# tlk00/BitMagic

Measured on AMD Instinct MI355X. Metric: Gbits/s + % HBM roofline, 256-way fused AND+COUNT on 1B-bit vectors, higher is better.
Workload: dtype u64; 1 GPU; aggregator pipeline combine_and_sub counts-only: 256-way AND+COUNT, 256 x 1000000000-bit vectors in total, data set A (common 10% OR noise 10%: no early exit); vectors=256, bits_per_vector=1000000000, density_q16=6554, blocks_per_vector=15259, blocks_per_rank=15259, hbm_resident_bytes=32279432448

## Files before the change

bitmagic_amd/__init__.py:

```python
from __future__ import annotations

import ctypes as C
from typing import Iterable, Sequence

import numpy as np

from . import _ffi
from ._ffi import BmxError, check, lib
from .sharding import shard_range, allreduce_counts

NULL, FULL, BIT, GAP = 0, 1, 2, 3
AND, OR, XOR, SUB = 0, 1, 2, 3
COUNT_AND, COUNT_XOR, COUNT_OR, COUNT_SUB_AB, COUNT_SUB_BA, COUNT_A, COUNT_B = 6, 7, 8, 9, 10, 11, 12
BLOCK_WORDS, BLOCK_BITS = 2048, 65536
opt_none, opt_compress = 0, 3
ID_MAX = 0xFFFFFFFF
ID_MAX64 = 0xFFFFFFFFFFFFFFFF
BM_UNSORTED, BM_SORTED, BM_SORTED_UNIFORM, BM_UNKNOWN = 0, 1, 2, 3

__all__ = ["context", "bvector", "aggregator", "slice_scanner", "rs_index", "rank_compressor", "group", "gbvector", "gaggregator", "gpipeline", "bit_import_u32", "count_and", "count_or",
           "count_xor", "count_sub", "distance_operation", "distance_matrix", "distance_matrix_dev",
           "COUNT_AND", "COUNT_XOR", "COUNT_OR", "COUNT_SUB_AB", "COUNT_SUB_BA", "COUNT_A", "COUNT_B", "BmxError", "simd_version", "device_count", "agg_run_options",
           "agg_opt_only_counts", "agg_opt_bvect_and_counts", "agg_opt_disable_bvects_and_counts",
           "BM_UNSORTED", "BM_SORTED", "BM_SORTED_UNIFORM", "BM_UNKNOWN"]
# ... 19 lines not shown
        self._h = C.c_void_p()
        check(lib().bmx_ctx_create(device, C.c_void_p(stream) if stream else None, C.byref(self._h)))
        self.device = device

    def close(self):
        if self._h:
            lib().bmx_ctx_destroy(self._h)
            self._h = C.c_void_p()

    def __del__(self):
        try:
            self.close()
        except Exception:
            pass

    def synchronize(self):
        check(lib().bmx_ctx_synchronize(self._h))

    def set_tuning(self, key: str, value: int):
        check(lib().bmx_ctx_set_tuning(self._h, key.encode(), int(value)))

    def trim(self):
        check(lib().bmx_ctx_trim(self._h))

    def redzone_check(self) -> dict:
        en, hits = C.c_int32(), C.c_uint64()
        buf = C.create_string_buffer(16384)
        check(lib().bmx_debug_redzone_check(self._h, C.byref(en), C.byref(hits), buf, len(buf)))
        return {"enabled": bool(en.value), "hits": hits.value, "report": buf.value.decode(errors="replace")}

    def inject_failure(self, kind: int, after: int = 0) -> None:
        check(lib().bmx_debug_inject_failure(self._h, int(kind), int(after)))

    def collection_prepare(self, vecs, role: int = 1) -> None:
        vecs = list(vecs)
        check(lib().bmx_collection_prepare(self._h, _handles(vecs), len(vecs), int(role)))

    def pack_stats(self) -> dict:
        n, b, ms = C.c_uint32(), C.c_uint64(), C.c_float()
        check(lib().bmx_ctx_pack_stats(self._h, C.byref(n), C.byref(b), C.byref(ms)))
        rb = C.c_uint64()
        check(lib().bmx_ctx_pack_run_bytes(self._h, C.byref(rb)))
        return {"collections": n.value, "bytes": b.value, "run_bytes": rb.value, "last_build_ms": ms.value}

    def mem_used(self) -> int:
        b = C.c_uint64()
# ... 1295 lines not shown
```

bitmagic_amd/_ffi.py:

```python
from __future__ import annotations

import ctypes as C
import os

_HERE = os.path.dirname(os.path.abspath(__file__))
LIB_PATH = os.environ.get("BMX_LIB") or os.path.join(_HERE, "lib", "libbmx.so")

OK, ERR_BADALLOC, ERR_BADARG, ERR_RANGE, ERR_DEVICE = 0, 1, 2, 3, 4


class BmxError(RuntimeError):
    def __init__(self, status: int, msg: str, detail: str):
        super().__init__(f"{msg}" + (f" [{detail}]" if detail else ""))
        self.status = status


_lib = None


def lib() -> C.CDLL:
    global _lib
    if _lib is not None:
        return _lib
    if not os.path.exists(LIB_PATH):
# ... 55 lines not shown
        "bmx_find_first_and_sub": (i32, [vp, P(vp), C.c_size_t, P(vp), C.c_size_t, P(i32), P(u64)]),
        "bmx_find_first_and_sub_range": (i32, [vp, P(vp), C.c_size_t, P(vp), C.c_size_t, u64, u64, P(i32), P(u64)]),
        "bmx_agg_shift_right_and": (i32, [vp, P(vp), C.c_size_t, i32, i32, P(vp), P(i32)]),
        "bmx_agg_shift_right_and_count": (i32, [vp, P(vp), C.c_size_t, P(u64)]),
        "bmx_slice_compare": (i32, [vp, P(vp), C.c_size_t, i32, u64, u64, u64, vp, P(vp), P(u64)]),
        "bmx_slice_compare_signed": (i32, [vp, P(vp), C.c_size_t, i32, C.c_int64, C.c_int64, u64, vp, P(vp), P(u64)]),
        "bmx_slice_compare_stat": (i32, [vp, P(vp), C.c_size_t, i32, u64, u64, u64, vp, P(u64), P(u64)]),
        "bmx_slice_eq_counts": (i32, [vp, P(vp), C.c_size_t, vp, C.c_size_t, u64, vp, vp]),
        "bmx_collection_prepare": (i32, [vp, P(vp), C.c_size_t, i32]),
        "bmx_ctx_pack_stats": (i32, [vp, P(u32), P(u64), P(C.c_float)]),
        "bmx_ctx_pack_run_bytes": (i32, [vp, P(u64)]),
        "bmx_pipeline_create": (i32, [vp, P(vp), P(u32), P(vp), P(u32), C.c_size_t, P(vp)]),
        "bmx_pipeline_destroy": (i32, [vp, vp]),
        "bmx_pipeline_set_search_count_limit": (i32, [vp, vp, u64]),
        "bmx_pipeline_last_windows": (i32, [vp, P(u32), P(u32)]),
        "bmx_pipeline_last_window_groups": (i32, [vp, P(u32), u32, P(u32)]),
        "bmx_pipeline_run_counts": (i32, [vp, vp, u32, u32, P(u64)]),
        "bmx_pipeline_run_counts_dev": (i32, [vp, vp, u32, u32, vp]),
        "bmx_pipeline_run_results": (i32, [vp, vp, P(vp), P(u64), vp, P(vp)]),
        "bmx_pipeline_run_results_range": (i32, [vp, vp, u32, u32, P(vp), P(u64), vp, P(vp)]),
        "bmx_pipeline_run_results_hint": (i32, [vp, vp, u64, u64, P(vp), P(u64), vp, P(vp)]),
        "bmx_pipeline_operand_bytes": (i32, [vp, vp, u32, u32, P(u64)]),
        "bmx_pipeline_describe": (i32, [vp, vp, u32, u32, C.c_char_p, C.c_size_t, P(u32)]),
        "bmx_rs_build": (i32, [vp, vp, P(vp)]),
        "bmx_rs_free": (i32, [vp, vp]),
        "bmx_rs_info": (i32, [vp, P(u64), P(i32)]),
        "bmx_rs_select_format": (i32, [vp, P(i32), P(u64)]),
        "bmx_rs_count": (i32, [vp, P(u64)]),
        "bmx_rs_export": (i32, [vp, vp, vp, vp]),
        "bmx_rank_batch": (i32, [vp, vp, vp, vp, C.c_size_t, vp]),
        "bmx_select_batch": (i32, [vp, vp, vp, vp, C.c_size_t, vp, vp]),
        "bmx_rank_batch_dev": (i32, [vp, vp, vp, vp, C.c_size_t, vp]),
        "bmx_select_batch_dev": (i32, [vp, vp, vp, vp, C.c_size_t, vp, vp]),
        "bmx_rank_compress": (i32, [vp, vp, vp, vp, i32, P(vp)]),
        "bmx_rank_decompress": (i32, [vp, vp, vp, vp, i32, P(vp)]),
        "bmx_rank_compress_many": (i32, [vp, vp, vp, P(vp), C.c_size_t, i32, P(vp)]),
        "bmx_rank_decompress_many": (i32, [vp, vp, vp, P(vp), C.c_size_t, i32, P(vp)]),
        "bmx_group_create": (i32, [P(i32), i32, i32, P(vp)]),
        "bmx_group_destroy": (i32, [vp]),
        "bmx_group_size": (i32, [vp, P(i32)]),
        "bmx_group_ctx": (i32, [vp, i32, P(vp)]),
        "bmx_group_shard_range": (i32, [vp, u32, i32, P(u32), P(u32)]),
        "bmx_block_table_weights": (i32, [u32, vp, vp, vp, u64, vp]),
        "bmx_group_partition_by_weight": (i32, [vp, u32, vp, vp]),
        "bmx_group_set_partition": (i32, [vp, u32, vp]),
        "bmx_group_rccl_ranks": (i32, [vp, P(i32)]),
# ... 67 lines not shown
```

bitmagic_amd/csrc/bmx.hip:

```cpp
#include "bmx_internal.h"
#ifdef BMX_DIAG
#include "bmx_diag.h"
#endif
#include "bmx_kernels2.h"
#include "bmx_kernels3.h"
#include "bmx_kernels4.h"
#include "bmx_kernels5.h"
#include "bmx_kernels6.h"
#include "bmx_kernels7.h"
#include "bmx_kernels8.h"
#include "bmx_kernels9.h"
#include "bmx_kernels10.h"
#include "bmx_kernels11.h"
#include "bmx_kernels12.h"
#include "bmx_kernels13.h"
#include "bmx_kernels14.h"
#include "bmx_kernels15.h"

#include <algorithm>
#include <atomic>
#include <chrono>
#include <cstdio>
#include <cstdlib>
#include <cstring>
// ... 627 lines not shown

static int coll_members_upload(bmx_ctx* ctx, const std::vector<u32>& ma, const std::vector<u32>& ms, DevBuf& d_buf, const u32** d_midx, const CollGroup** d_groups)
{
    const size_t nm = ma.size() + ms.size(), goff = (nm * 4 + 15) & ~(size_t)15;
    std::vector<u8> h(goff + sizeof(CollGroup));
    if (!ma.empty()) memcpy(h.data(), ma.data(), ma.size() * 4);
    if (!ms.empty()) memcpy(h.data() + ma.size() * 4, ms.data(), ms.size() * 4);
    const CollGroup g{0u, (u32)ma.size(), (u32)ma.size(), (u32)ms.size()};
    memcpy(h.data() + goff, &g, sizeof(g));
    int rc;
    if ((rc = dmalloc(ctx, &d_buf.p, h.size())) || (rc = h2d_staged(ctx, d_buf.p, h.data(), h.size()))) { d_buf.reset(); return rc; }
    *d_midx = (const u32*)d_buf.p; *d_groups = (const CollGroup*)((const char*)d_buf.p + goff);
    return BMX_OK;
}

static bool use_split(const bmx_ctx* ctx, const bmx_pipeline* p, u64 nitems)
{
    if (ctx->pipe_split == 0 || !nitems) return false;
    if (ctx->pipe_split == 1) return nitems <= 65535u * 16u;
    return nitems <= 384u && (u64)p->n_ops >= 24ull * p->ngroups;
}
#define SPLIT_WAVES 8

typedef void (*pipe_bits_fn)(const u64*, const u32*, const u32*, u32, u32, u32, u32, int, u64*);

static u32 pipe_window_cap(u32 wg)
{
    u32 wpb = wg / 64u;
    u32 per_cu = wpb >= 7u ? 1u : 12u / wpb;
    return 256u * per_cu * wpb;
}
static void pipe_plan(const bmx_ctx* ctx, u64 nitems, u32 ngroups, u32& rows, u32& wg, u32& unroll, u32& window)
{
    rows = (u32)ctx->pipe_rows;
    if (!rows) rows = nitems >= 1400u ? 8u : nitems >= 700u ? 4u : nitems >= 350u ? 2u : 1u;
    unroll = ctx->pipe_unroll ? (u32)ctx->pipe_unroll : ((rows >= 4u || !ctx->pipe_nt) ? 4u : 8u);
    u64 n = nitems * (8u / rows);
    wg = (u32)ctx->pipe_wg;
    if (!wg) {
        wg = 256u;
        if (rows == 8u) {
            static const u32 cand[3] = {640u, 768u, 512u};
            double best = -1.0;
            for (u32 c : cand) {
                u64 cap = pipe_window_cap(c), nwin = (n + cap - 1) / cap, per = (n + nwin - 1) / nwin;
                double fill = (double)per / (double)cap;
                if (fill > best + 0.02) { best = fill; wg = c; }
// ... 19 lines not shown
        if (unroll == 4 && nt) switch (wg) { case 384: return B2(4, true, 384); case 512: return B2(4, true, 512);
                                             case 640: return B2(4, true, 640); case 768: return B2(4, true, 768); default: break; }
        if (unroll == 4 && !nt && wg == 512) return B2(4, false, 512);
    }
#ifdef BMX_TUNE
    if constexpr (ROWS == 8) {
        if (nt && unroll == 4) switch (wg) { case 192: return B2(4, true, 192); case 320: return B2(4, true, 320); case 448: return B2(4, true, 448);
                                             case 576: return B2(4, true, 576); default: break; }
        if (nt && unroll == 2) switch (wg) { case 256: return B2(2, true, 256); case 384: return B2(2, true, 384); case 640: return B2(2, true, 640);
                                             case 1024: return B2(2, true, 1024); default: break; }
        if (nt && unroll == 1 && wg == 256) return B2(1, true, 256);
    } else {
        if (nt && wg == 384) {
            if (unroll == 4) return B2(4, true, 384);
            if constexpr (ROWS <= 4) { if (unroll == 8) return B2(8, true, 384); }
            if constexpr (ROWS <= 2) { if (unroll == 16) return B2(16, true, 384); }
        }
        if (nt && wg == 512 && unroll == 4) return B2(4, true, 512);
    }
#endif
#undef B2
    return nullptr;
}
static pipe_bits_fn pipe_bits_kernel(u32 rows, u32 unroll, bool nt, u32 wg)
{
    switch (rows) {
    case 8: return pipe_bits_rows<8>(unroll, nt, wg);
    case 4: return pipe_bits_rows<4>(unroll, nt, wg);
    case 2: return pipe_bits_rows<2>(unroll, nt, wg);
    case 1: return pipe_bits_rows<1>(unroll, nt, wg);
    default: return nullptr;
    }
}

static int ctx_set_tuning(bmx_ctx* ctx, const char* key, int value)
{
    ARGCHK(ctx && key);
    std::string k(key);
    if (k == "pipe_unroll") { ARGCHK(value == 0 || value == 1 || value == 2 || value == 4 || value == 8 || value == 16); ctx->pipe_unroll = value; }
    else if (k == "pipe_rows") { ARGCHK(value == 0 || value == 8 || value == 4 || value == 2 || value == 1); ctx->pipe_rows = value; }
    else if (k == "pipe_nt") ctx->pipe_nt = value != 0;
    else if (k == "pipe_lds") { ARGCHK(value >= 0 && value <= 160 * 1024); ctx->pipe_lds = value; }
    else if (k == "pipe_slots") { ARGCHK(value == 8 || value == 16); ctx->pipe_slots = value; }
    else if (k == "pipe_staged") { ARGCHK(value >= -1 && value <= 1); ctx->pipe_staged = value; }
    else if (k == "pipe_split") { ARGCHK(value >= -1 && value <= 1); ctx->pipe_split = value; }
    else if (k == "pipe_window") { ARGCHK(value >= -1); ctx->pipe_window = value; }
    else if (k == "or_tile") { ARGCHK(value >= 0 && value <= 3); ctx->or_tile = value; }
    else if (k == "or_rows") { ARGCHK(value >= -1 && value <= 1); ctx->or_rows = value; }
    else if (k == "or_depth") { ARGCHK(value == 4 || value == 8); ctx->or_depth = value; }
    else if (k == "direct_cols") { ARGCHK(value >= 0); ctx->direct_cols = value; }
    else if (k == "pair_stream") { ARGCHK(value == -1 || value == 0 || value == 2 || value == 4 || value == 8); ctx->pair_stream = value; }
    else if (k == "pair_wgs") { ARGCHK(value >= 1 && value <= 8); ctx->pair_wgs = value; }
    else if (k == "range_halves") { ARGCHK(value == 0 || value == 1); ctx->range_halves = value; }
    else if (k == "gap_count") { ARGCHK(value >= -1 && value <= 1); ctx->gap_count = value; }
    else if (k == "agg_shape") { ARGCHK(value == 0 || value == 1); ctx->agg_shape = value; }
    else if (k == "and_rows") { ARGCHK(value >= -1 && value <= 1); ctx->and_rows = value; }
    else if (k == "and_rows_wg") { ARGCHK(value == 128 || value == 256 || value == 512); ctx->and_rows_wg = value; }
    else if (k == "and_rows_depth") { ARGCHK(value == 2 || value == 3 || value == 4 || value == 8); ctx->and_rows_depth = value; }
    else if (k == "and_rows_nt") ctx->and_rows_nt = value != 0;
    else if (k == "and_rows_ipw") { ARGCHK(value >= 0 && value <= 64); ctx->and_rows_ipw = value; }
    else if (k == "ff_window") { ARGCHK(value >= -1); ctx->ff_window = value; }
    else if (k == "or_window") { ARGCHK(value >= -9); ctx->or_window = value; }
    else if (k == "gap_pack") { ARGCHK(value >= -1 && value <= 1); ctx->gap_pack = value; }
    else if (k == "coll_members") { ARGCHK(value >= -1 && value <= 1); ctx->coll_members = value; ++ctx->coll_gen; }
    else if (k == "coll_shape") { ARGCHK(value >= 0 && value <= 5); ctx->coll_shape = value; }
    else if (k == "op2_nt") { ARGCHK(value >= 0 && value <= 3); ctx->op2_nt = value; }
    else if (k == "op2_loop") { ARGCHK(value >= -1 && value <= 8); ctx->op2_loop = value; }
    else if (k == "op2_wgs") { ARGCHK(value >= 1 && value <= 8); ctx->op2_wgs = value; }
    else if (k == "pair_nt") { ARGCHK(value >= 0 && value <= 1); ctx->pair_nt = value; }
// ... 60 lines not shown
    dfree(ctx, p->scratch);
    const int rc = p->v ? vec_release(p->v) : BMX_OK;
    delete p;
    return rc;
}
void ctx_release(bmx_ctx* ctx)
{
    (void)hipSetDevice(ctx->device);
    if (ctx->stream) (void)hipStreamSynchronize(ctx->stream);
    while (!ctx->colls.empty()) coll_free(ctx, ctx->colls.size() - 1);
    pool_trim(ctx);
    rz_verify(ctx, nullptr);
    if (ctx->rz_hits) fprintf(stderr, "[bmx redzone] context destroyed with %llu damaged allocation(s) found during its life\n", (unsigned long long)ctx->rz_hits);
    for (auto& kv : ctx->pool_live) { auto rz = ctx->rz_live.find(kv.first); (void)hipFree(rz != ctx->rz_live.end() ? rz->second.raw : kv.first); if (rz != ctx->rz_live.end()) ctx->rz_live.erase(rz); }
    ctx->pool_live.clear();
    ensure_release(ctx, &ctx->scratch, &ctx->scratch_bytes);
    ensure_release(ctx, &ctx->aux, &ctx->aux_bytes);
    if (ctx->d_small) (void)hipFree(ctx->d_small);
    if (ctx->d_slots) (void)hipFree(ctx->d_slots);
    if (ctx->d_done) (void)hipFree(ctx->d_done);
    if (ctx->d_slots2) (void)hipFree(ctx->d_slots2);
    if (ctx->d_done2) (void)hipFree(ctx->d_done2);
    if (ctx->d_cursor) (void)hipFree(ctx->d_cursor);
    if (ctx->h_pend) (void)hipHostFree(ctx->h_pend);
    if (ctx->d_zero) (void)hipFree(ctx->d_zero);
    if (ctx->h_small) (void)hipHostFree(ctx->h_small);
    if (ctx->h_stage) (void)hipHostFree(ctx->h_stage);
    if (ctx->ev_stage) (void)hipEventDestroy(ctx->ev_stage);
    if (ctx->ev0) (void)hipEventDestroy(ctx->ev0);
    if (ctx->ev1) (void)hipEventDestroy(ctx->ev1);
    if (ctx->own_stream && ctx->stream) (void)hipStreamDestroy(ctx->stream);
    delete ctx;
}

extern "C" {

const char* bmx_error_msg(int status)
{
    switch (status) {
    case BMX_OK: return "BMX-00: All correct";
    case BMX_ERR_BADALLOC: return "BMX-01: Allocation error (HBM or host)";
    case BMX_ERR_BADARG: return "BMX-02: Invalid or missing function argument";
    case BMX_ERR_RANGE: return "BMX-03: Incorrect range or index";
    case BMX_ERR_DEVICE: return "BMX-04: No usable gfx950 device or HIP runtime failure";
    default: return "BMX-XX: Unknown error";
    }
// ... 20 lines not shown
    Owned<bmx_ctx> ctx(new bmx_ctx());
    ctx->device = device;
    if (stream) ctx->stream = (hipStream_t)stream;
    else { HIPCHK(hipStreamCreateWithFlags(&ctx->stream, hipStreamNonBlocking)); ctx->own_stream = true; }
    HIPCHK(hipEventCreate(&ctx->ev0));
    HIPCHK(hipEventCreate(&ctx->ev1));
    HIPCHK(hipMalloc((void**)&ctx->d_small, 64 * sizeof(u64)));
    HIPCHK(hipHostMalloc((void**)&ctx->h_small, 64 * sizeof(u64)));
    HIPCHK(hipHostMalloc((void**)&ctx->h_stage, STAGE_BYTES));
    HIPCHK(hipEventCreateWithFlags(&ctx->ev_stage, hipEventDisableTiming));
    HIPCHK(hipMalloc((void**)&ctx->d_slots, COUNT_SLOTS * COUNT_SLOT_STRIDE * sizeof(u64)));
    HIPCHK(hipMemsetAsync(ctx->d_slots, 0, COUNT_SLOTS * COUNT_SLOT_STRIDE * sizeof(u64), ctx->stream));
    HIPCHK(hipMalloc((void**)&ctx->d_zero, 256));
    HIPCHK(hipMemsetAsync(ctx->d_zero, 0, 256, ctx->stream));
    HIPCHK(hipMalloc((void**)&ctx->d_done, FOLD_DONE_WORDS * 4));
    HIPCHK(hipMemsetAsync(ctx->d_done, 0, FOLD_DONE_WORDS * 4, ctx->stream));
    HIPCHK(hipMalloc((void**)&ctx->d_slots2, COUNT_SLOTS * COUNT_SLOT_STRIDE * sizeof(u64)));
    HIPCHK(hipMemsetAsync(ctx->d_slots2, 0, COUNT_SLOTS * COUNT_SLOT_STRIDE * sizeof(u64), ctx->stream));
    HIPCHK(hipMalloc((void**)&ctx->d_done2, FOLD_DONE_WORDS * 4));
    HIPCHK(hipMemsetAsync(ctx->d_done2, 0, FOLD_DONE_WORDS * 4, ctx->stream));
    HIPCHK(hipHostMalloc((void**)&ctx->h_pend, PEND_SLOTS * 8 * sizeof(u64)));
    HIPCHK(hipMalloc((void**)&ctx->d_cursor, 64));
    HIPCHK(hipMemsetAsync(ctx->d_cursor, 0, 64, ctx->stream));
    { int v = 0; if (hipDeviceGetAttribute(&v, hipDeviceAttributeMaxSharedMemoryPerBlock, device) == hipSuccess && v > 0) ctx->max_lds_bytes = (uint32_t)v; else (void)hipGetLastError(); }
    { size_t fr = 0, tot = 0; if (hipMemGetInfo(&fr, &tot) == hipSuccess && fr) ctx->pack_cap = (uint64_t)fr / 4; else (void)hipGetLastError(); }
    if (const char* e = getenv("BMX_DEBUG_REDZONE")) ctx->redzone = atoi(e) != 0;
    if (const char* e = getenv("BMX_PACK_MAX_MB")) { long long mb = atoll(e); if (mb >= 0) ctx->pack_cap = (uint64_t)mb << 20; }
    if (const char* e = getenv("BMX_POOL_MAX_MB")) { long long mb = atoll(e); if (mb >= 0) ctx->pool_cap = (uint64_t)mb << 20; }
    static const char* const env_keys[][2] = {
        {"BMX_PIPE_UNROLL", "pipe_unroll"}, {"BMX_PIPE_ROWS", "pipe_rows"}, {"BMX_PIPE_NT", "pipe_nt"},
        {"BMX_PIPE_WG", "pipe_wg"}, {"BMX_PIPE_WINDOW", "pipe_window"}, {"BMX_PIPE_SPLIT", "pipe_split"}, {"BMX_OR_TILE", "or_tile"}, {"BMX_OR_ROWS", "or_rows"}, {"BMX_OR_DEPTH", "or_depth"}, {"BMX_OR_WINDOW", "or_window"}, {"BMX_DIRECT_COLS", "direct_cols"}, {"BMX_FF_WINDOW", "ff_window"}, {"BMX_GAP_COUNT", "gap_count"}, {"BMX_AND_ROWS", "and_rows"}, {"BMX_AGG_SHAPE", "agg_shape"}, {"BMX_AND_ROWS_WG", "and_rows_wg"}, {"BMX_AND_ROWS_DEPTH", "and_rows_depth"}, {"BMX_AND_ROWS_NT", "and_rows_nt"}, {"BMX_AND_ROWS_IPW", "and_rows_ipw"}, {"BMX_RANGE_HALVES", "range_halves"}, {"BMX_PAIR_STREAM", "pair_stream"}, {"BMX_PAIR_WGS", "pair_wgs"}, {"BMX_RS_LANES", "rs_lanes"}, {"BMX_RS_SELECT_TOP", "rs_select_top"}, {"BMX_RS_SELECT_SEL", "rs_select_sel"}, {"BMX_RS_LINES", "rs_lines"}, {"BMX_RS_SELECT_LINES", "rs_select_lines"}, {"BMX_RS_SDIR_SHIFT", "rs_sdir_shift"}, {"BMX_COLL_SHAPE", "coll_shape"}, {"BMX_COLL_WINDOW", "coll_window"}, {"BMX_COLL_SPLIT", "coll_split"}, {"BMX_COLL_BUILD", "coll_build"}, {"BMX_EQ_BIG", "eq_big"}, {"BMX_PAIR_LOOP", "pair_loop"}, {"BMX_PAIR_NT", "pair_nt"}, {"BMX_EQ_BIG_SHAPE", "eq_big_shape"}, {"BMX_OP2_WGS", "op2_wgs"}, {"BMX_OP2_LOOP", "op2_loop"}, {"BMX_OP2_NT", "op2_nt"}, {"BMX_GAP_PACK", "gap_pack"}, {"BMX_COLL_MEMBERS", "coll_members"}, {"BMX_XCD_SWIZZLE", "xcd_swizzle"}, {"BMX_RANKC_PATH", "rankc_path"}};
    for (auto& kv : env_keys)
        if (const char* e = getenv(kv[0])) (void)ctx_set_tuning(ctx.get(), kv[1], atoi(e));
    g_last_error.clear();
    *out = ctx.release();
    return BMX_OK;
ABI_END }

int bmx_ctx_destroy(bmx_ctx* ctx) { ABI_TRY if (ctx) ctx_release(ctx); return BMX_OK; ABI_END }

int bmx_ctx_set_tuning(bmx_ctx* ctx, const char* key, int value) { ABI_TRY return ctx_set_tuning(ctx, key, value); ABI_END }

int bmx_probe_stream_rw(bmx_ctx* ctx, uint64_t bytes, int sets, int wgs_per_cu, int iters, float* ms_per_pass)
{ ABI_TRY
    ARGCHK(ctx && ms_per_pass && bytes >= 8192 && sets >= 1 && sets <= 8 && wgs_per_cu >= 1 && wgs_per_cu <= 8 && iters >= 1);
    int rc = set_dev(ctx); if (rc) return rc;
    const u64 nblk = bytes / 8192;
    if (nblk > 0x7FFFFFFFull) { g_last_error = "probe buffer too large"; return BMX_ERR_RANGE; }
    void* buf = nullptr;
    HIPCHK(hipMalloc(&buf, (size_t)nblk * 8192 * 3 * sets));
    hipError_t e = hipMemsetAsync(buf, 0x5A, (size_t)nblk * 8192 * 3 * sets, ctx->stream);
    const u32 waves = 4u, total = 256u * waves * (u32)wgs_per_cu;
    const u32 per_wave = (u32)((nblk + total - 1u) / total);
    const u32 grid = (u32)(((nblk + per_wave - 1u) / per_wave + waves - 1u) / waves);
// ... 1169 lines not shown
        }
    }
    if (use_split(ctx, p, nitems64)) {
        size_t lds = (size_t)SPLIT_WAVES * 8192;
        auto fn = k_pipe_split<2, SPLIT_WAVES>;
        HIPCHK(hipFuncSetAttribute(reinterpret_cast<const void*>(fn), hipFuncAttributeMaxDynamicSharedMemorySize, (int)lds));
        hipLaunchKernelGGL(fn, dim3((u32)nitems64), dim3(SPLIT_WAVES * 64), lds, ctx->stream,
                           (const u64*)p->d_dmat, row_off, and_n, sub_n, p->col_stride, ngroups, nb_from, nb_to, 0, (u64*)d_counts,
                           0, (uint4*)nullptr, (u64*)nullptr, (BlockStat*)nullptr);
        KCHK();
        return BMX_OK;
    }
    if (!p->has_gap) {
        u32 rows, wg, unroll, window;
        pipe_plan(ctx, nitems64, ngroups, rows, wg, unroll, window);
        u32 parts = 8u / rows;
        if (nitems64 * parts > 0xFFFFFFF0ull) { g_last_error = "too many work items in one run"; return BMX_ERR_RANGE; }
        pipe_bits_fn fn = pipe_bits_kernel(rows, unroll, ctx->pipe_nt != 0, wg);
        if (!fn) { g_last_error = "this (pipe_rows, pipe_unroll, pipe_nt, pipe_wg) shape is not compiled into the library"; return BMX_ERR_BADARG; }
        u32 wpb = wg / 64u;
        u32 ncols = nb_to - nb_from;
        u32 nwin = window ? (ncols + window - 1u) / window : 1u;
        u32 per = (ncols + nwin - 1u) / nwin;
        for (u32 c0 = 0; c0 < ncols; c0 += per) {
            u32 cols = std::min(per, ncols - c0);
            u32 nitems = cols * ngroups * parts, grid = (nitems + wpb - 1) / wpb;
            hipLaunchKernelGGL(fn, dim3(grid), dim3(wg), (size_t)ctx->pipe_lds, ctx->stream,
                               (const u64*)p->d_dmat, row_off, and_n, p->col_stride, ngroups, nb_from + c0, nitems, ctx->xcd_swz, (u64*)d_counts);
            KCHK();
        }
        return BMX_OK;
    }
    if (nitems64 > 0xFFFFFFF0ull) { g_last_error = "too many (column, group) items in one run"; return BMX_ERR_RANGE; }
    if (use_and_rows(ctx, p)) {
        const u32 ipw = ctx->and_rows_ipw > 0 ? (u32)ctx->and_rows_ipw : 1u;
        hipLaunchKernelGGL(and_rows_kernel<AR_COUNT>(ctx), dim3((u32)((nitems64 + ipw - 1u) / ipw)), dim3((u32)ctx->and_rows_wg), 0, ctx->stream,
                           (const u64*)p->d_dmat, row_off, and_n, sub_n, p->col_stride, ngroups, nb_from, (u32)nitems64, ctx->xcd_swz, (u64*)d_counts,
                           (uint4*)nullptr, (u64*)nullptr, (BlockStat*)nullptr, 0u, 0xFFFFFFFFu, and_rows_diag_bits(), ipw);
        KCHK();
        return BMX_OK;
    }
    if (use_gapcount(ctx, p)) {
        size_t lds = (size_t)(16384 * 2 + 2048) * 4;
        HIPCHK(hipFuncSetAttribute(reinterpret_cast<const void*>(k_pipe_counts_gapcount<false>), hipFuncAttributeMaxDynamicSharedMemorySize, (int)lds));
        hipLaunchKernelGGL(HIP_KERNEL_NAME(k_pipe_counts_gapcount<false>), dim3((u32)nitems64), dim3(1024), lds, ctx->stream,
                           p->d_dmat, row_off, and_n, sub_n, p->col_stride, ngroups, nb_from, (u32)nitems64, (u64*)d_counts,
                           (uint4*)nullptr, (u64*)nullptr, (BlockStat*)nullptr, 0u, 0xFFFFFFFFu);
        KCHK();
        return BMX_OK;
    }
    size_t lds = 4 * 2048 * 4;
// ... 35 lines not shown
        snprintf(buf, buf_len, "k_pipe_split<2,%d> x 1 launch, %llu workgroups", SPLIT_WAVES, (unsigned long long)nitems64);
    else if (use_and_rows(ctx, p))
        snprintf(buf, buf_len, "k_agg_and_rows<COUNT,%d,%d> x 1 launch, %llu workgroups", ctx->and_rows_wg, ctx->and_rows_depth, (unsigned long long)nitems64);
    else if (use_gapcount(ctx, p))
        snprintf(buf, buf_len, "k_pipe_counts_gapcount x 1 launch, %llu workgroups", (unsigned long long)nitems64);
    else if (p->has_gap)
        snprintf(buf, buf_len, "k_pipe_counts<%d> x 1 launch", ctx->pipe_unroll == 1 ? 1 : ctx->pipe_unroll == 2 ? 2 : 4);
    else {
        u32 rows, wg, unroll, window;
        pipe_plan(ctx, nitems64, p->ngroups, rows, wg, unroll, window);
        u32 ncols = nb_to - nb_from, nwin = (window && ncols) ? (ncols + window - 1u) / window : 1u;
        u32 per = nwin ? (ncols + nwin - 1u) / nwin : 0u;
        snprintf(buf, buf_len, "k_pipe_counts_bits2<%u,%s,%u,%u> x %u launch%s of <= %u columns", unroll, ctx->pipe_nt ? "true" : "false",
                 wg, rows, nwin, nwin == 1 ? "" : "es", per);
        if (n_launches) *n_launches = nwin;
    }
    return BMX_OK;
ABI_END }

int bmx_pipeline_set_search_count_limit(bmx_ctx* ctx, bmx_pipeline* p, uint64_t limit)
{ ABI_TRY
    ARGCHK(ctx && p && p->ctx == ctx);
    p->search_limit = (limit == 0 || limit == 0xFFFFFFFFull || limit == 0xFFFFFFFFFFFFull) ? ~0ull : limit;
    return BMX_OK;
ABI_END }

int bmx_pipeline_last_windows(const bmx_pipeline* p, uint32_t* launched, uint32_t* planned)
{ ABI_TRY
    ARGCHK(p);
    if (launched) *launched = p->last_windows;
    if (planned) *planned = p->last_windows_planned;
    return BMX_OK;
ABI_END }

}

static int limit_counts_run(bmx_ctx* ctx, bmx_pipeline* p, uint32_t nb_from, uint32_t nb_to, uint64_t* counts_out)
{
    int rc;
    uint32_t f = nb_from, t = nb_to;
    if ((rc = pipe_range(p, f, t))) return rc;
    const u32 ng = p->ngroups, ncols = t - f;
    p->h_win_groups.clear(); p->h_stop.assign(ng, 0xFFFFFFFFu);
    u32 w = std::max<u32>(ncols / 64u, 16u), planned = 0;
    for (u32 c = 0, ww = w; c < ncols; c += ww, ww *= 4u) ++planned;
    p->last_windows_planned = std::max(planned, 1u); p->last_windows = 0;
// ... 2003 lines not shown
```

bitmagic_amd/csrc/bmx_device.h:

```cpp
#pragma once
#include <hip/hip_runtime.h>
#include <stdint.h>

typedef uint8_t  u8;
typedef uint16_t u16;
typedef uint32_t u32;
typedef uint64_t u64;

#define GMETA(e) ((u32)((e) >> 48) & 0x1FFFu)
#define GMETA_NONE 0xFFFFFFFFu
#define BMX_DESC_KIND(d) ((u32)((d) & 3ull))
#define BMX_DESC_PTR(d)  ((d) & ~3ull)

typedef u32 u32x4 __attribute__((ext_vector_type(4)));
typedef const __attribute__((address_space(1))) u32x4* gcptr4;
typedef __attribute__((address_space(1))) u32x4* gptr4;
typedef const __attribute__((address_space(1))) u16* gcptr16;

template <int ROWS> struct Part { u32x4 r[ROWS]; };
typedef Part<8> Blk;

__device__ __forceinline__ gcptr4 as_gc4(u64 addr) { return (gcptr4)(uintptr_t)addr; }
__device__ __forceinline__ gcptr4 as_gc4(const void* p) { return (gcptr4)(uintptr_t)p; }
__device__ __forceinline__ gptr4 as_g4(void* p) { return (gptr4)(uintptr_t)p; }
// ... 690 lines not shown
            for (int i = 0; i < ROWS; ++i) {
                if constexpr (OPK == 0) acc.r[i] &= buf[u].r[i];
                else if constexpr (OPK == 1) acc.r[i] &= ~buf[u].r[i];
                else acc.r[i] |= buf[u].r[i];
            }
        if constexpr (OPK == 2) return part_is_ones<ROWS>(acc); else return part_is_zero<ROWS>(acc);
    };
    Part<ROWS> A[U], B[U];
    u32 k = U;
    fetch(0);
    issue(A);
    fetch(k);
    bool zero;
    do {
        issue(B); fetch(k + U);
        bool z1 = consume(A);
        issue(A); fetch(k + 2 * U);
        bool z2 = consume(B);
        zero = z1 | z2;
        k += 2 * U;
    } while (!zero && k < n + U);
    return zero;
}
```

bitmagic_amd/csrc/bmx_internal.h:

```cpp
#pragma once
#include "../../include/bmx.h"
#include <hip/hip_runtime.h>
#include <stdint.h>

#include <map>
#include <memory>
#include <string>
#include <unordered_map>
#include <vector>

typedef uint8_t  u8;
typedef uint16_t u16;
typedef uint32_t u32;
typedef uint64_t u64;

int bmx_fail_hip(hipError_t e, const char* what, const char* file, int line);
void bmx_set_last_error(const char* msg);
#define HIPCHK(call) do { hipError_t e_ = (call); if (e_ != hipSuccess) return bmx_fail_hip(e_, #call, __FILE__, __LINE__); } while (0)
#define ARGCHK(cond) do { if (!(cond)) { bmx_set_last_error("bad argument: " #cond); return BMX_ERR_BADARG; } } while (0)
#define KCHK() HIPCHK(hipGetLastError())
#define PEND_SLOTS 1024
#include <new>
#include <stdexcept>
int bmx_abi_caught(int kind, const char* what);
// ... 16 lines not shown
    u64* d_slots = nullptr;
    u64* d_slots2 = nullptr; u32* d_done2 = nullptr;
    u64* h_pend = nullptr; uint64_t pend_used[16] = {};
    u64* d_cursor = nullptr;
    u64* d_zero = nullptr;
    u32* d_done = nullptr;
    u64* h_small = nullptr;
    char* h_stage = nullptr; size_t stage_off = 0;
    hipEvent_t ev_stage = nullptr;
    std::multimap<size_t, void*> pool_free;
    std::unordered_map<void*, size_t> pool_live;
    uint64_t pool_cached = 0, pool_cap = 16ull << 30;
    struct RzInfo { void* raw; size_t block; size_t bytes; int line; };
    bool redzone = false;
    std::unordered_map<void*, RzInfo> rz_live;
    uint64_t rz_hits = 0; std::string rz_report;
    long long fail_dmalloc_after = -1;
    bool fail_dmalloc_throws = false;
    int pipe_unroll = 0;
    int pipe_rows = 0;
    int pipe_nt = 1;
    int pipe_wg = 0;
    int pipe_window = 0;
    int pipe_staged = -1;
    int pipe_lds = 0;
    int pipe_slots = 16;
    int pipe_split = -1;
    int or_tile = 0;
    int direct_cols = 384;
    int pair_stream = -1;
    int pair_wgs = 1;
    int range_halves = 1;
    int gap_count = -1;
    int agg_shape = 0;
    int and_rows = -1;
    int and_rows_wg = 256;
    int and_rows_ipw = 0;
    int and_rows_nt = 0;
    int and_rows_depth = 3;
    int ff_window = 0;
    int or_window = 0;
    int or_rows = -1;
    int or_depth = 4;
    std::vector<struct bmx_coll*> colls;
    int gap_pack = -1;
    uint64_t pack_cap = 16ull << 30, pack_bytes = 0, coll_tick = 0;
// ... 130 lines not shown
```

bitmagic_amd/csrc/bmx_kernels.h:

```cpp
#pragma once
#include "bmx_device.h"

#define DESC_MAKE(ptr, kind) ((u64)(uintptr_t)(ptr) | ((u64)(kind) << 62))
#define DESC_K(d) ((u32)((d) >> 62))
#define DESC_P(d) ((d) & 0x0000FFFFFFFFFFFFull)
#define DESC_MAKE_GAP(ptr, len, sbit) (DESC_MAKE(ptr, K_GAP) | ((u64)((((u32)(len)) << 1) | ((u32)(sbit) & 1u)) << 48))
enum { K_NULL = 0, K_FULL = 1, K_BIT = 2, K_GAP = 3 };

#define ROW_EMPTY 1ull
#define ROW_FULL  2ull
#define ROW_ONES  4ull

struct BlockStat { u32 pop; u32 runs; u32 first; u32 kind; };

__global__ __launch_bounds__(256)
void k_generate(u64 seed, u32 vec_id, int with_common, u32 d, u64 nbits, u64* __restrict__ out, u64 nwords64, u64 word0)
{
    u64 i = (u64)blockIdx.x * blockDim.x + threadIdx.x;
    u64 stride = (u64)gridDim.x * blockDim.x;
    for (; i < nwords64; i += stride) {
        u64 w = word0 + i;
        u64 v = gen_word64(seed, vec_id, w, d);
        if (with_common) v |= gen_word64(seed, 0xFFFFFFFFu, w, d);
        u64 bit0 = w * 64u;
// ... 377 lines not shown
    u32 na = uniform32(and_n[g]), ns = uniform32(sub_n[g]);
    const u64* pa = row + 2;
    const u64* ps = pa + na;
    u32* lds = lds_dyn + wave * 2048u;

    Blk acc;
    blk_fill(acc, ~0u);
    if (pipe_chain<U, true, 0>(acc, pa, nba, lane)) return;
    if (pipe_chain<U, true, 1>(acc, ps, nbs, lane)) return;
    if (nga | ngs) {
        blk_to_lds(acc, lds, lane);
        if (nga && gap_apply_list<GAP_AND>(pa + na - 1u, nga, lds, lane)) return;
        if (ngs && gap_apply_list<GAP_SUB>(ps + ns - 1u, ngs, lds, lane)) return;
        blk_from_lds(acc, lds, lane);
    }
    u32 cnt = wave_sum(blk_lane_popcount(acc));
    if (lane == 0 && cnt) atomicAdd(reinterpret_cast<unsigned long long*>(&counts[g]), (unsigned long long)cnt);
}

template <int U, bool NT, int WG = 256, int ROWS = 8>
__global__ __launch_bounds__(WG)
void k_pipe_counts_bits2(const u64* __restrict__ dmat, const u32* __restrict__ row_off,
                         const u32* __restrict__ and_n, u32 col_stride,
                         u32 ngroups, u32 col_from, u32 nitems, int xcd_swz, u64* __restrict__ counts)
{
    constexpr u32 PARTS = 8 / ROWS;
    u32 lane = lane_id(), wave = threadIdx.x >> 6, wpb = blockDim.x >> 6;
    u32 bid = xcd_swz ? xcd_remap(blockIdx.x, gridDim.x) : blockIdx.x;
    u32 item = uniform32(bid * wpb + wave);
    if (item >= nitems) return;
    u32 part = item % PARTS, cg = item / PARTS;
    u32 c = cg / ngroups, g = cg - c * ngroups;
    const u64* row = dmat + (size_t)(col_from + c) * col_stride + row_off[g];
    u64 hdr = uniform64(row[0]), flags = uniform64(row[1]);
    if (flags & ROW_EMPTY) return;
    if (flags & ROW_FULL) { if (lane == 0) atomicAdd(reinterpret_cast<unsigned long long*>(&counts[g]), (unsigned long long)(65536u / PARTS)); return; }
    u32 nba = (u32)(hdr & 0xFFFFu), nbs = (u32)((hdr >> 32) & 0xFFFFu);
    u32 na = uniform32(and_n[g]);
    const u64* pa = row + 2;
    const u64* ps = pa + na;
    const u32 poff = part * ROWS * 64u;
    Part<ROWS> acc;
#pragma unroll
    for (int i = 0; i < ROWS; ++i) acc.r[i] = (u32x4)(~0u);
    if (pipe_chain<U, NT, 0, ROWS>(acc, pa, nba, lane, poff)) return;
    if (pipe_chain<U, NT, 1, ROWS>(acc, ps, nbs, lane, poff)) return;
    u32 cnt = 0;
#pragma unroll
    for (int i = 0; i < ROWS; ++i) {
        cnt += __popcll(((u64)acc.r[i].y << 32) | acc.r[i].x);
        cnt += __popcll(((u64)acc.r[i].w << 32) | acc.r[i].z);
    }
    cnt = wave_sum(cnt);
    if (lane == 0 && cnt) atomicAdd(reinterpret_cast<unsigned long long*>(&counts[g]), (unsigned long long)cnt);
}

#ifdef BMX_DIAG
template <int AUX>
__global__ __launch_bounds__(256)
void k_diag_stream_read_buf(const uint4* __restrict__ buf, u64 nblocks8k, u32 blocks_per_wave, int pattern, int xcd_swz, u64* __restrict__ sink)
{
    u32 lane = lane_id();
    u32 bid = xcd_swz ? xcd_remap(blockIdx.x, gridDim.x) : blockIdx.x;
    u64 w = (u64)bid * (blockDim.x >> 6) + (threadIdx.x >> 6);
    u64 nwaves = nblocks8k / blocks_per_wave;
    if (w >= nwaves) return;
    u64 b0 = pattern ? w : w * blocks_per_wave;
    u64 step = pattern ? nwaves : 1;
    u32x4 acc = (u32x4)(0u);
// ... 60 lines not shown
```

include/bmx.h:

```cpp
#ifndef BMX_H
#define BMX_H

#include <stddef.h>
#include <stdint.h>

#ifdef __cplusplus
extern "C" {
#endif

#define BMX_OK            0
#define BMX_ERR_BADALLOC  1
#define BMX_ERR_BADARG    2
#define BMX_ERR_RANGE     3
#define BMX_ERR_DEVICE    4

#define BMX_NULL 0
#define BMX_FULL 1
#define BMX_BIT  2
#define BMX_GAP  3

#define BMX_AND 0
#define BMX_OR  1
#define BMX_XOR 2
#define BMX_SUB 3
// ... 125 lines not shown
int bmx_pipeline_create(bmx_ctx* ctx,
                        const bmx_vec* const* and_list, const uint32_t* and_n,
                        const bmx_vec* const* sub_list, const uint32_t* sub_n,
                        size_t ngroups, bmx_pipeline** out);
int bmx_pipeline_destroy(bmx_ctx* ctx, bmx_pipeline* p);
int bmx_pipeline_run_counts(bmx_ctx* ctx, bmx_pipeline* p, uint32_t nb_from, uint32_t nb_to,
                            uint64_t* counts_out);
int bmx_pipeline_set_search_count_limit(bmx_ctx* ctx, bmx_pipeline* p, uint64_t limit);
int bmx_pipeline_last_windows(const bmx_pipeline* p, uint32_t* launched, uint32_t* planned);
int bmx_pipeline_last_window_groups(const bmx_pipeline* p, uint32_t* out, uint32_t cap, uint32_t* n);
int bmx_pipeline_run_counts_dev(bmx_ctx* ctx, bmx_pipeline* p, uint32_t nb_from, uint32_t nb_to,
                                uint64_t* d_counts);
int bmx_pipeline_run_results(bmx_ctx* ctx, bmx_pipeline* p, bmx_vec** results_out, uint64_t* counts_out,
                             const bmx_vec* or_target_in, bmx_vec** or_target_out);
int bmx_pipeline_run_results_range(bmx_ctx* ctx, bmx_pipeline* p, uint32_t nb_from, uint32_t nb_to, bmx_vec** results_out,
                                   uint64_t* counts_out, const bmx_vec* or_target_in, bmx_vec** or_target_out);
int bmx_pipeline_run_results_hint(bmx_ctx* ctx, bmx_pipeline* p, uint64_t from, uint64_t to, bmx_vec** results_out,
                                  uint64_t* counts_out, const bmx_vec* or_target_in, bmx_vec** or_target_out);
int bmx_pipeline_operand_bytes(bmx_ctx* ctx, bmx_pipeline* p, uint32_t nb_from, uint32_t nb_to,
                               uint64_t* bytes);

int bmx_pipeline_describe(bmx_ctx* ctx, bmx_pipeline* p, uint32_t nb_from, uint32_t nb_to, char* buf, size_t buf_len,
                          uint32_t* n_launches);

int bmx_rs_build(bmx_ctx* ctx, const bmx_vec* v, bmx_rs** out);
int bmx_rs_free(bmx_ctx* ctx, bmx_rs* rs);
int bmx_rs_info(const bmx_rs* rs, uint64_t* bytes, int* has_lines);
int bmx_rs_select_format(const bmx_rs* rs, int* offset_bits, uint64_t* bytes);
int bmx_rs_count(const bmx_rs* rs, uint64_t* count);
int bmx_rs_export(bmx_ctx* ctx, const bmx_rs* rs, uint32_t* bcount, uint64_t* sub_count);
int bmx_rank_batch(bmx_ctx* ctx, const bmx_vec* v, const bmx_rs* rs,
                   const uint64_t* n, size_t q, uint64_t* out);
int bmx_select_batch(bmx_ctx* ctx, const bmx_vec* v, const bmx_rs* rs,
                     const uint64_t* rank, size_t q, uint64_t* pos, uint8_t* found);
int bmx_rank_batch_dev(bmx_ctx* ctx, const bmx_vec* v, const bmx_rs* rs,
                       const uint64_t* d_n, size_t q, uint64_t* d_out);
int bmx_select_batch_dev(bmx_ctx* ctx, const bmx_vec* v, const bmx_rs* rs,
                         const uint64_t* d_rank, size_t q, uint64_t* d_pos, uint8_t* d_found);

int bmx_rank_compress(bmx_ctx* ctx, const bmx_vec* idx, const bmx_rs* rs_idx, const bmx_vec* src, int optimize, bmx_vec** out);
int bmx_rank_decompress(bmx_ctx* ctx, const bmx_vec* idx, const bmx_rs* rs_idx, const bmx_vec* src, int optimize, bmx_vec** out);
int bmx_rank_compress_many(bmx_ctx* ctx, const bmx_vec* idx, const bmx_rs* rs_idx, const bmx_vec* const* srcs, size_t n,
                           int optimize, bmx_vec** outs);
int bmx_rank_decompress_many(bmx_ctx* ctx, const bmx_vec* idx, const bmx_rs* rs_idx, const bmx_vec* const* srcs, size_t n,
                             int optimize, bmx_vec** outs);

// ... 79 lines not shown
```

Baseline: 55630 Gbit/s.

## Narrow AND chain to live stripes using masked buffer loads

After folding the first U operands, the pipeline counts kernel checks how many 16-byte stripes of the accumulator are still nonzero. If that is at or below a threshold, it switches to a narrow loop where lanes with dead stripes issue out-of-range buffer loads, so those reads are dropped by the hardware. This aims to cut HBM traffic for blocks that become sparse early without reaching all-zero. It adds ballot and popcount overhead per step and smaller load batches, and it only helps when the intermediate AND becomes sparse within a stripe. Optional counters record how often narrowing happens.

```diff
diff --git a/bitmagic_amd/__init__.py b/bitmagic_amd/__init__.py
--- a/bitmagic_amd/__init__.py
+++ b/bitmagic_amd/__init__.py
@@ -65,6 +65,11 @@
 
     def trim(self):
         check(lib().bmx_ctx_trim(self._h))
+
+    def narrow_stat(self) -> tuple:
+        out = (C.c_uint64 * 2)()
+        check(lib().bmx_pipeline_narrow_stat(self._h, out))
+        return int(out[0]), int(out[1])
 
     def redzone_check(self) -> dict:
         en, hits = C.c_int32(), C.c_uint64()
diff --git a/bitmagic_amd/_ffi.py b/bitmagic_amd/_ffi.py
--- a/bitmagic_amd/_ffi.py
+++ b/bitmagic_amd/_ffi.py
@@ -101,6 +101,7 @@
         "bmx_pipeline_run_results_hint": (i32, [vp, vp, u64, u64, P(vp), P(u64), vp, P(vp)]),
         "bmx_pipeline_operand_bytes": (i32, [vp, vp, u32, u32, P(u64)]),
         "bmx_pipeline_describe": (i32, [vp, vp, u32, u32, C.c_char_p, C.c_size_t, P(u32)]),
+        "bmx_pipeline_narrow_stat": (i32, [vp, P(u64)]),
         "bmx_rs_build": (i32, [vp, vp, P(vp)]),
         "bmx_rs_free": (i32, [vp, vp]),
         "bmx_rs_info": (i32, [vp, P(u64), P(i32)]),
diff --git a/bitmagic_amd/csrc/bmx.hip b/bitmagic_amd/csrc/bmx.hip
--- a/bitmagic_amd/csrc/bmx.hip
+++ b/bitmagic_amd/csrc/bmx.hip
@@ -673,7 +673,7 @@
 }
 #define SPLIT_WAVES 8
 
-typedef void (*pipe_bits_fn)(const u64*, const u32*, const u32*, u32, u32, u32, u32, int, u64*);
+typedef void (*pipe_bits_fn)(const u64*, const u32*, const u32*, u32, u32, u32, u32, int, u64*, u32, u64*);
 
 static u32 pipe_window_cap(u32 wg)
 {
@@ -739,6 +739,12 @@
 #undef B2
     return nullptr;
 }
+#define PIPE_NARROW_AUTO 16
+static u32 pipe_narrow_thr(const bmx_ctx* ctx, u32 rows)
+{
+    const u32 per_block = ctx->pipe_narrow < 0 ? (u32)PIPE_NARROW_AUTO : (u32)ctx->pipe_narrow;
+    return (per_block * rows + 7u) / 8u;
+}
 static pipe_bits_fn pipe_bits_kernel(u32 rows, u32 unroll, bool nt, u32 wg)
 {
     switch (rows) {
@@ -762,6 +768,7 @@
     else if (k == "pipe_staged") { ARGCHK(value >= -1 && value <= 1); ctx->pipe_staged = value; }
     else if (k == "pipe_split") { ARGCHK(value >= -1 && value <= 1); ctx->pipe_split = value; }
     else if (k == "pipe_window") { ARGCHK(value >= -1); ctx->pipe_window = value; }
+    else if (k == "pipe_narrow") { ARGCHK(value >= -1 && value <= 64); ctx->pipe_narrow = value; }
     else if (k == "or_tile") { ARGCHK(value >= 0 && value <= 3); ctx->or_tile = value; }
     else if (k == "or_rows") { ARGCHK(value >= -1 && value <= 1); ctx->or_rows = value; }
     else if (k == "or_depth") { ARGCHK(value == 4 || value == 8); ctx->or_depth = value; }
@@ -868,6 +875,7 @@
     if (ctx->d_slots2) (void)hipFree(ctx->d_slots2);
     if (ctx->d_done2) (void)hipFree(ctx->d_done2);
     if (ctx->d_cursor) (void)hipFree(ctx->d_cursor);
+    if (ctx->d_nstat) (void)hipFree(ctx->d_nstat);
     if (ctx->h_pend) (void)hipHostFree(ctx->h_pend);
     if (ctx->d_zero) (void)hipFree(ctx->d_zero);
     if (ctx->h_small) (void)hipHostFree(ctx->h_small);
@@ -934,6 +942,8 @@
     HIPCHK(hipHostMalloc((void**)&ctx->h_pend, PEND_SLOTS * 8 * sizeof(u64)));
     HIPCHK(hipMalloc((void**)&ctx->d_cursor, 64));
     HIPCHK(hipMemsetAsync(ctx->d_cursor, 0, 64, ctx->stream));
+    HIPCHK(hipMalloc((void**)&ctx->d_nstat, 2 * sizeof(u64)));
+    HIPCHK(hipMemsetAsync(ctx->d_nstat, 0, 2 * sizeof(u64), ctx->stream));
     { int v = 0; if (hipDeviceGetAttribute(&v, hipDeviceAttributeMaxSharedMemoryPerBlock, device) == hipSuccess && v > 0) ctx->max_lds_bytes = (uint32_t)v; else (void)hipGetLastError(); }
     { size_t fr = 0, tot = 0; if (hipMemGetInfo(&fr, &tot) == hipSuccess && fr) ctx->pack_cap = (uint64_t)fr / 4; else (void)hipGetLastError(); }
     if (const char* e = getenv("BMX_DEBUG_REDZONE")) ctx->redzone = atoi(e) != 0;
@@ -941,7 +951,7 @@
     if (const char* e = getenv("BMX_POOL_MAX_MB")) { long long mb = atoll(e); if (mb >= 0) ctx->pool_cap = (uint64_t)mb << 20; }
     static const char* const env_keys[][2] = {
         {"BMX_PIPE_UNROLL", "pipe_unroll"}, {"BMX_PIPE_ROWS", "pipe_rows"}, {"BMX_PIPE_NT", "pipe_nt"},
-        {"BMX_PIPE_WG", "pipe_wg"}, {"BMX_PIPE_WINDOW", "pipe_window"}, {"BMX_PIPE_SPLIT", "pipe_split"}, {"BMX_OR_TILE", "or_tile"}, {"BMX_OR_ROWS", "or_rows"}, {"BMX_OR_DEPTH", "or_depth"}, {"BMX_OR_WINDOW", "or_window"}, {"BMX_DIRECT_COLS", "direct_cols"}, {"BMX_FF_WINDOW", "ff_window"}, {"BMX_GAP_COUNT", "gap_count"}, {"BMX_AND_ROWS", "and_rows"}, {"BMX_AGG_SHAPE", "agg_shape"}, {"BMX_AND_ROWS_WG", "and_rows_wg"}, {"BMX_AND_ROWS_DEPTH", "and_rows_depth"}, {"BMX_AND_ROWS_NT", "and_rows_nt"}, {"BMX_AND_ROWS_IPW", "and_rows_ipw"}, {"BMX_RANGE_HALVES", "range_halves"}, {"BMX_PAIR_STREAM", "pair_stream"}, {"BMX_PAIR_WGS", "pair_wgs"}, {"BMX_RS_LANES", "rs_lanes"}, {"BMX_RS_SELECT_TOP", "rs_select_top"}, {"BMX_RS_SELECT_SEL", "rs_select_sel"}, {"BMX_RS_LINES", "rs_lines"}, {"BMX_RS_SELECT_LINES", "rs_select_lines"}, {"BMX_RS_SDIR_SHIFT", "rs_sdir_shift"}, {"BMX_COLL_SHAPE", "coll_shape"}, {"BMX_COLL_WINDOW", "coll_window"}, {"BMX_COLL_SPLIT", "coll_split"}, {"BMX_COLL_BUILD", "coll_build"}, {"BMX_EQ_BIG", "eq_big"}, {"BMX_PAIR_LOOP", "pair_loop"}, {"BMX_PAIR_NT", "pair_nt"}, {"BMX_EQ_BIG_SHAPE", "eq_big_shape"}, {"BMX_OP2_WGS", "op2_wgs"}, {"BMX_OP2_LOOP", "op2_loop"}, {"BMX_OP2_NT", "op2_nt"}, {"BMX_GAP_PACK", "gap_pack"}, {"BMX_COLL_MEMBERS", "coll_members"}, {"BMX_XCD_SWIZZLE", "xcd_swizzle"}, {"BMX_RANKC_PATH", "rankc_path"}};
+        {"BMX_PIPE_WG", "pipe_wg"}, {"BMX_PIPE_WINDOW", "pipe_window"}, {"BMX_PIPE_NARROW", "pipe_narrow"}, {"BMX_PIPE_SPLIT", "pipe_split"}, {"BMX_OR_TILE", "or_tile"}, {"BMX_OR_ROWS", "or_rows"}, {"BMX_OR_DEPTH", "or_depth"}, {"BMX_OR_WINDOW", "or_window"}, {"BMX_DIRECT_COLS", "direct_cols"}, {"BMX_FF_WINDOW", "ff_window"}, {"BMX_GAP_COUNT", "gap_count"}, {"BMX_AND_ROWS", "and_rows"}, {"BMX_AGG_SHAPE", "agg_shape"}, {"BMX_AND_ROWS_WG", "and_rows_wg"}, {"BMX_AND_ROWS_DEPTH", "and_rows_depth"}, {"BMX_AND_ROWS_NT", "and_rows_nt"}, {"BMX_AND_ROWS_IPW", "and_rows_ipw"}, {"BMX_RANGE_HALVES", "range_halves"}, {"BMX_PAIR_STREAM", "pair_stream"}, {"BMX_PAIR_WGS", "pair_wgs"}, {"BMX_RS_LANES", "rs_lanes"}, {"BMX_RS_SELECT_TOP", "rs_select_top"}, {"BMX_RS_SELECT_SEL", "rs_select_sel"}, {"BMX_RS_LINES", "rs_lines"}, {"BMX_RS_SELECT_LINES", "rs_select_lines"}, {"BMX_RS_SDIR_SHIFT", "rs_sdir_shift"}, {"BMX_COLL_SHAPE", "coll_shape"}, {"BMX_COLL_WINDOW", "coll_window"}, {"BMX_COLL_SPLIT", "coll_split"}, {"BMX_COLL_BUILD", "coll_build"}, {"BMX_EQ_BIG", "eq_big"}, {"BMX_PAIR_LOOP", "pair_loop"}, {"BMX_PAIR_NT", "pair_nt"}, {"BMX_EQ_BIG_SHAPE", "eq_big_shape"}, {"BMX_OP2_WGS", "op2_wgs"}, {"BMX_OP2_LOOP", "op2_loop"}, {"BMX_OP2_NT", "op2_nt"}, {"BMX_GAP_PACK", "gap_pack"}, {"BMX_COLL_MEMBERS", "coll_members"}, {"BMX_XCD_SWIZZLE", "xcd_swizzle"}, {"BMX_RANKC_PATH", "rankc_path"}};
     for (auto& kv : env_keys)
         if (const char* e = getenv(kv[0])) (void)ctx_set_tuning(ctx.get(), kv[1], atoi(e));
     g_last_error.clear();
@@ -2157,11 +2167,13 @@
         u32 ncols = nb_to - nb_from;
         u32 nwin = window ? (ncols + window - 1u) / window : 1u;
         u32 per = (ncols + nwin - 1u) / nwin;
+        const u32 narrow_thr = pipe_narrow_thr(ctx, rows);
+        u64* nstat = ctx->narrow_armed ? ctx->d_nstat : nullptr;
         for (u32 c0 = 0; c0 < ncols; c0 += per) {
             u32 cols = std::min(per, ncols - c0);
             u32 nitems = cols * ngroups * parts, grid = (nitems + wpb - 1) / wpb;
             hipLaunchKernelGGL(fn, dim3(grid), dim3(wg), (size_t)ctx->pipe_lds, ctx->stream,
-                               (const u64*)p->d_dmat, row_off, and_n, p->col_stride, ngroups, nb_from + c0, nitems, ctx->xcd_swz, (u64*)d_counts);
+                               (const u64*)p->d_dmat, row_off, and_n, p->col_stride, ngroups, nb_from + c0, nitems, ctx->xcd_swz, (u64*)d_counts, narrow_thr, nstat);
             KCHK();
         }
         return BMX_OK;
@@ -2243,6 +2255,19 @@
 { ABI_TRY
     ARGCHK(ctx && p && p->ctx == ctx);
     p->search_limit = (limit == 0 || limit == 0xFFFFFFFFull || limit == 0xFFFFFFFFFFFFull) ? ~0ull : limit;
+    return BMX_OK;
+ABI_END }
+
+int bmx_pipeline_narrow_stat(bmx_ctx* ctx, uint64_t out[2])
+{ ABI_TRY
+    ARGCHK(ctx && out);
+    int rc = set_dev(ctx); if (rc) return rc;
+    out[0] = out[1] = 0;
+    if (!ctx->narrow_armed) { ctx->narrow_armed = true; return BMX_OK; }
+    HIPCHK(hipMemcpyAsync(ctx->h_small, ctx->d_nstat, 2 * sizeof(u64), hipMemcpyDeviceToHost, ctx->stream));
+    HIPCHK(hipMemsetAsync(ctx->d_nstat, 0, 2 * sizeof(u64), ctx->stream));
+    HIPCHK(hipStreamSynchronize(ctx->stream));
+    out[0] = ctx->h_small[0]; out[1] = ctx->h_small[1];
     return BMX_OK;
 ABI_END }
 
diff --git a/bitmagic_amd/csrc/bmx_device.h b/bitmagic_amd/csrc/bmx_device.h
--- a/bitmagic_amd/csrc/bmx_device.h
+++ b/bitmagic_amd/csrc/bmx_device.h
@@ -736,3 +736,87 @@
     } while (!zero && k < n + U);
     return zero;
 }
+
+template <int ROWS>
+__device__ __forceinline__ u32 part_live_stripes(const Part<ROWS>& acc)
+{
+    u32 live = 0;
+#pragma unroll
+    for (int i = 0; i < ROWS; ++i) {
+        u64 m = __ballot((acc.r[i].x | acc.r[i].y | acc.r[i].z | acc.r[i].w) != 0u);
+        m |= m >> 4; m |= m >> 2; m |= m >> 1;
+        live += (u32)__popcll(m & 0x0101010101010101ull);
+    }
+    return uniform32(live);
+}
+
+template <int U, bool NT, int OPK, int ROWS>
+__device__ __forceinline__ bool pipe_narrow(Part<ROWS>& acc, const u64* __restrict__ plist, u32 n, u32 lane, u32 poff, bool stat, u32& pieces)
+{
+    constexpr int NB = (ROWS == 8 && U > 2) ? U / 2 : U;
+#pragma unroll 1
+    for (u32 k = 0; k < n; k += NB) {
+        u64 pn[NB];
+#pragma unroll
+        for (int u = 0; u < NB; ++u) pn[u] = plist[k + u < n ? k + u : n - 1u];
+        if (stat) {
+            u32 np = 0;
+#pragma unroll
+            for (int i = 0; i < ROWS; ++i) np += (u32)__popcll(__ballot((acc.r[i].x | acc.r[i].y | acc.r[i].z | acc.r[i].w) != 0u));
+            pieces += (u32)NB * np;
+        }
+        __amdgpu_buffer_rsrc_t rs[NB];
+#pragma unroll
+        for (int u = 0; u < NB; ++u)
+            rs[u] = __builtin_amdgcn_make_buffer_rsrc((void*)(uintptr_t)(uniform64(pn[u]) + (u64)poff * 16u), 0, ROWS * 1024, 0x00020000);
+        Part<ROWS> buf[NB];
+#pragma unroll
+        for (int i = 0; i < ROWS; ++i) {
+            const bool live = (acc.r[i].x | acc.r[i].y | acc.r[i].z | acc.r[i].w) != 0u;
+            const int voff = live ? (int)(lane * 16u) : (int)0x80000000u;
+#pragma unroll
+            for (int u = 0; u < NB; ++u) buf[u].r[i] = __builtin_amdgcn_raw_buffer_load_b128(rs[u], voff, i * 1024, NT ? 2 : 0);
+        }
+#pragma unroll
+        for (int u = 0; u < NB; ++u)
+#pragma unroll
+            for (int i = 0; i < ROWS; ++i) {
+                if constexpr (OPK == 0) acc.r[i] &= buf[u].r[i]; else acc.r[i] &= ~buf[u].r[i];
+            }
+        if (part_is_zero<ROWS>(acc)) return true;
+    }
+    return false;
+}
+
+template <int U, bool NT, int OPK, int ROWS>
+__device__ __forceinline__ bool pipe_fold(Part<ROWS>& acc, const u64* __restrict__ plist, u32 n, u32 lane, u32 poff, u32 thr,
+                                          bool stat, bool& narrowed, u32& pieces)
+{
+    static_assert(OPK == 0 || OPK == 1, "the OR chain does not narrow");
+    if (n == 0) return false;
+    u32 done = 0;
+    bool sparse = thr != 0u && part_live_stripes<ROWS>(acc) <= thr;
+    if (thr != 0u && !sparse) {
+        u64 pn[U];
+#pragma unroll
+        for (int u = 0; u < U; ++u) pn[u] = plist[(u32)u < n ? (u32)u : n - 1u];
+        Part<ROWS> buf[U];
+#pragma unroll
+        for (int u = 0; u < U; ++u) part_load<ROWS, NT>(buf[u], as_gc4(uniform64(pn[u])) + poff, lane);
+#pragma unroll
+        for (int u = 0; u < U; ++u)
+#pragma unroll
+            for (int i = 0; i < ROWS; ++i) {
+                if constexpr (OPK == 0) acc.r[i] &= buf[u].r[i]; else acc.r[i] &= ~buf[u].r[i];
+            }
+        const u32 live = part_live_stripes<ROWS>(acc);
+        if (live == 0u) return true;
+        if (n <= (u32)U) return false;
+        sparse = live <= thr;
+        done = (u32)U;
+    }
+    if (sparse) narrowed = true;
+    if (pipe_narrow<U, NT, OPK, ROWS>(acc, plist + done, sparse ? n - done : 0u, lane, poff, stat, pieces)) return true;
+    if (sparse) return false;
+    return pipe_chain<U, NT, OPK, ROWS>(acc, plist + done, n - done, lane, poff);
+}
diff --git a/bitmagic_amd/csrc/bmx_internal.h b/bitmagic_amd/csrc/bmx_internal.h
--- a/bitmagic_amd/csrc/bmx_internal.h
+++ b/bitmagic_amd/csrc/bmx_internal.h
@@ -62,6 +62,8 @@
     int pipe_nt = 1;
     int pipe_wg = 0;
     int pipe_window = 0;
+    int pipe_narrow = -1;
+    u64* d_nstat = nullptr; bool narrow_armed = false;
     int pipe_staged = -1;
     int pipe_lds = 0;
     int pipe_slots = 16;
diff --git a/bitmagic_amd/csrc/bmx_kernels.h b/bitmagic_amd/csrc/bmx_kernels.h
--- a/bitmagic_amd/csrc/bmx_kernels.h
+++ b/bitmagic_amd/csrc/bmx_kernels.h
@@ -423,7 +423,8 @@
 __global__ __launch_bounds__(WG)
 void k_pipe_counts_bits2(const u64* __restrict__ dmat, const u32* __restrict__ row_off,
                          const u32* __restrict__ and_n, u32 col_stride,
-                         u32 ngroups, u32 col_from, u32 nitems, int xcd_swz, u64* __restrict__ counts)
+                         u32 ngroups, u32 col_from, u32 nitems, int xcd_swz, u64* __restrict__ counts,
+                         u32 narrow_thr, u64* __restrict__ nstat)
 {
     constexpr u32 PARTS = 8 / ROWS;
     u32 lane = lane_id(), wave = threadIdx.x >> 6, wpb = blockDim.x >> 6;
@@ -444,8 +445,16 @@
     Part<ROWS> acc;
 #pragma unroll
     for (int i = 0; i < ROWS; ++i) acc.r[i] = (u32x4)(~0u);
-    if (pipe_chain<U, NT, 0, ROWS>(acc, pa, nba, lane, poff)) return;
-    if (pipe_chain<U, NT, 1, ROWS>(acc, ps, nbs, lane, poff)) return;
+    const bool stat = nstat != nullptr;
+    bool narrowed = false;
+    u32 pieces = 0;
+    bool zero = pipe_fold<U, NT, 0, ROWS>(acc, pa, nba, lane, poff, narrow_thr, stat, narrowed, pieces);
+    if (!zero) zero = pipe_fold<U, NT, 1, ROWS>(acc, ps, nbs, lane, poff, narrow_thr, stat, narrowed, pieces);
+    if (stat && narrowed && lane == 0) {
+        atomicAdd(reinterpret_cast<unsigned long long*>(&nstat[0]), 1ull);
+        atomicAdd(reinterpret_cast<unsigned long long*>(&nstat[1]), (unsigned long long)pieces);
+    }
+    if (zero) return;
     u32 cnt = 0;
 #pragma unroll
     for (int i = 0; i < ROWS; ++i) {
diff --git a/include/bmx.h b/include/bmx.h
--- a/include/bmx.h
+++ b/include/bmx.h
@@ -171,6 +171,7 @@
 
 int bmx_pipeline_describe(bmx_ctx* ctx, bmx_pipeline* p, uint32_t nb_from, uint32_t nb_to, char* buf, size_t buf_len,
                           uint32_t* n_launches);
+int bmx_pipeline_narrow_stat(bmx_ctx* ctx, uint64_t out[2]);
 
 int bmx_rs_build(bmx_ctx* ctx, const bmx_vec* v, bmx_rs** out);
 int bmx_rs_free(bmx_ctx* ctx, bmx_rs* rs);
```

Measured after the change: 54610 Gbit/s. 0.982x the previous value.
